# sony/timbre-trap

Hardware: AMD Instinct MI355X
Metric: audio-seconds/s training throughput (9oct x 60bpo, 3s@22.05kHz) (higher is better)
Workload: dtype bf16; 1 GPU; full train step (CQT x2 + AE fwd/bwd with consistency + 3 losses + clip + AdamW), model_complexity=2 latent=128, 64 clips x 3 s per GPU, under torch.autocast like reference experiments/train.py:415 (bf16 MFMA conv path of BASELINE config[2]; fp32 master weights, losses and optimizer); global_batch=64, parallelism=dp1

## Files before the change

timbre-trap_amd/csrc/latent_bf16.hip:

```cpp
#include "bf16_common.h"

namespace {

#ifndef LAT_WGRAD_WAVES
#define LAT_WGRAD_WAVES 4
#endif
#ifndef LAT_EXPAND_Q
#define LAT_EXPAND_Q 2
#endif
#ifndef LAT_NSPLIT
#define LAT_NSPLIT 32
#endif

__device__ __forceinline__ float gate_f(float dy, float y) { return dy * elu_dout(y); }

template <int CT> __device__ __forceinline__ int ochc(int ct, int m) { return (CT / 4) * (m >> 2) + 4 * ct + (m & 3); }

template <int CT, int DT>
__global__ __launch_bounds__(NT) void k_lat_wprep1(const float* __restrict__ w, e16* __restrict__ wp, int D, int E) {
    constexpr int SPH = CT / 32;
    const int i = blockIdx.x * NT + threadIdx.x;
    if (i >= E * SPH * DT * 64) return;
    const int lane = i & 63, dt = (i >> 6) % DT, s = (i >> 6) / DT;
    const int h = s / SPH, half = s - h * SPH;
    const int d = 16 * dt + (lane & 15), c0 = 32 * half + 8 * (lane >> 4);
    e16x8 v;
#pragma unroll
    for (int e = 0; e < 8; ++e) v[e] = (e16)(d < D ? w[((long)d * CT + c0 + e) * E + h] : 0.f);
    reinterpret_cast<e16x8*>(wp)[i] = v;
}
template <int CT, int KS>
__global__ __launch_bounds__(NT) void k_lat_wprep2(const float* __restrict__ w, e16* __restrict__ wp, int D, int E) {
    constexpr int NC = CT / 16;
    const int i = blockIdx.x * NT + threadIdx.x;
    if (i >= E * NC * KS * 64) return;
    const int lane = i & 63, s = (i >> 6) % KS, ct = ((i >> 6) / KS) % NC, h = (i >> 6) / (KS * NC);
    const int c = ochc<CT>(ct, lane & 15), d0 = 32 * s + 8 * (lane >> 4);
    e16x8 v;
#pragma unroll
    for (int e = 0; e < 8; ++e) v[e] = (e16)(d0 + e < D ? w[((long)(d0 + e) * CT + c) * E + h] : 0.f);
    reinterpret_cast<e16x8*>(wp)[i] = v;
}
template <int KS>
__global__ __launch_bounds__(NT) void k_lat_zprep(const float* __restrict__ z, e16* __restrict__ zt, int D, int Dz, float fill, int T,
                                                   long npix, float zscale, int one_row = -1) {
    constexpr int ZS = 32 * KS + 16, PCS = ZS / 8;
    const long i = (long)blockIdx.x * NT + threadIdx.x;
    const long pix = (i / (64 * PCS)) * 64 + (i & 63);
    if (pix >= npix) return;
    const int d0 = (int)((i >> 6) % PCS) * 8;
    const long b = pix / T, t = pix - b * T;
    e16x8 v;
#pragma unroll
    for (int e = 0; e < 8; ++e)
        v[e] = (e16)(zscale * (d0 + e < Dz ? z[(b * Dz + d0 + e) * T + t] : (d0 + e < D ? fill : (d0 + e == one_row ? 1.f : 0.f))));
    *reinterpret_cast<e16x8*>(zt + pix * ZS + d0) = v;
}

template <int CT, int DT, bool GATE, int QN>
__global__ __launch_bounds__(NT) void k_lat_contract(const e16* __restrict__ in, const e16* __restrict__ gy,
                                                      const e16* __restrict__ wp, const float* __restrict__ bias,
                                                      float* __restrict__ out, int D, int Dout, int E, int T, long npix, float oscale) {
    constexpr int SPH = CT / 32;
    constexpr int CHUNK = DT * 64 * 16, ROUNDS = (DT * 64 + NT - 1) / NT;
    extern __shared__ __align__(16) unsigned char smem[];
    const int tid = threadIdx.x, lane = tid & 63, wave = tid >> 6;
    const int n = lane & 15, g = lane >> 4;
    const int nsteps = E * SPH;
    const long p0 = (long)blockIdx.x * (64 * QN) + wave * (16 * QN);
    long pix[QN]; bool ok[QN]; long base[QN];
#pragma unroll
    for (int q = 0; q < QN; ++q) {
        pix[q] = p0 + 16 * q + n;
        ok[q] = pix[q] < npix;
        const long b = pix[q] / T, t = pix[q] - b * T;
        base[q] = (b * E * T + t) * CT + 8 * g;
    }
    auto stage = [&](int s, int buf) {
        const e16* src = wp + (long)s * (DT * 64 * 8);
#pragma unroll
        for (int r = 0; r < ROUNDS; ++r) {
            const int i = r * NT + wave * 64, p = i + lane;
            glds16(src + (long)(p < DT * 64 ? p : DT * 64 - 1) * 8, smem + buf * (ROUNDS * NT * 16) + (long)i * 16);
        }
    };
    auto fetch = [&](int s, e16x8 (&q8)[QN]) {
        const int h = s / SPH, half = s - h * SPH;
#pragma unroll
        for (int q = 0; q < QN; ++q) {
            const long off = base[q] + (long)h * T * CT + 32 * half;
            const bool live = ok[q] && s < nsteps;
            e16x8 v = *reinterpret_cast<const e16x8*>(in + (live ? off : 0));
            if (GATE) {
                const e16x8 yv = *reinterpret_cast<const e16x8*>(gy + (live ? off : 0));
#pragma unroll
                for (int e = 0; e < 8; ++e) v[e] = (e16)gate_f((float)v[e], (float)yv[e]);
            }
            if (!live)
#pragma unroll
                for (int e = 0; e < 8; ++e) v[e] = (e16)0.f;
            q8[q] = v;
        }
    };
    f32x4 acc[DT][QN];
#pragma unroll
    for (int dt = 0; dt < DT; ++dt)
#pragma unroll
        for (int q = 0; q < QN; ++q) acc[dt][q] = f32x4{0.f, 0.f, 0.f, 0.f};
    e16x8 bq[QN], bn[QN];
    stage(0, 0);
    fetch(0, bq);
    for (int s = 0; s < nsteps; ++s) {
        asm volatile("s_waitcnt vmcnt(0)" ::: "memory");
        __syncthreads();
        if (s + 1 < nsteps) stage(s + 1, (s + 1) & 1);
        fetch(s + 1, bn);
        const unsigned char* wb = smem + (s & 1) * (ROUNDS * NT * 16);
#pragma unroll
        for (int dt = 0; dt < DT; ++dt) {
            const e16x8 a = *reinterpret_cast<const e16x8*>(wb + ((long)dt * 64 + lane) * 16);
#pragma unroll
            for (int q = 0; q < QN; ++q) acc[dt][q] = mma32(a, bq[q], acc[dt][q]);
        }
#pragma unroll
        for (int q = 0; q < QN; ++q) bq[q] = bn[q];
    }
#pragma unroll
    for (int q = 0; q < QN; ++q) {
        if (!ok[q]) continue;
        const long b = pix[q] / T, t = pix[q] - b * T;
#pragma unroll
        for (int dt = 0; dt < DT; ++dt)
#pragma unroll
            for (int r = 0; r < 4; ++r) {
                const int d = 16 * dt + 4 * g + r;
                if (d < Dout) out[(b * Dout + d) * T + t] = acc[dt][q][r] * oscale + (bias ? bias[d] : 0.f);
            }
    }
    (void)CHUNK;
}

template <int CT, int KS, bool ACT, int QE, bool GOUT = false>
__global__ __launch_bounds__(NT) void k_lat_expand(const e16* __restrict__ zt, const e16* __restrict__ wp,
                                                    const float* __restrict__ bias, e16* __restrict__ out, int E, int T,
                                                    long npix, const e16* __restrict__ gy = nullptr) {
    constexpr int NC = CT / 16, NCH = CT / 4, ZS = 32 * KS + 16;
    constexpr int PCS = NC * KS * 64, ROUNDS = (PCS + NT - 1) / NT;
    extern __shared__ __align__(16) unsigned char smem[];
    const int tid = threadIdx.x, lane = tid & 63, wave = tid >> 6;
    const int n = lane & 15, g = lane >> 4;
    const long p0 = (long)blockIdx.x * (64 * QE) + wave * (16 * QE);
    e16x8 bz[QE][KS];
    long obase[QE]; bool ok[QE];
#pragma unroll
    for (int q = 0; q < QE; ++q) {
        const long pix = p0 + 16 * q + n;
        ok[q] = pix < npix;
        const long pc = ok[q] ? pix : 0;
#pragma unroll
        for (int s = 0; s < KS; ++s) bz[q][s] = *reinterpret_cast<const e16x8*>(zt + pc * ZS + 32 * s + 8 * g);
        const long b = pc / T, t = pc - b * T;
        obase[q] = (b * E * T + t) * CT + NCH * g;
    }
    float br[NCH];
#pragma unroll
    for (int e = 0; e < NCH; ++e) br[e] = ACT ? bias[NCH * g + e] : 0.f;
    auto stage = [&](int h, int buf) {
        const e16* src = wp + (long)h * (PCS * 8);
#pragma unroll
        for (int r = 0; r < ROUNDS; ++r) {
            const int i = r * NT + wave * 64, p = i + lane;
            glds16(src + (long)(p < PCS ? p : PCS - 1) * 8, smem + buf * (ROUNDS * NT * 16) + (long)i * 16);
        }
    };
    stage(0, 0);
    for (int h = 0; h < E; ++h) {
        asm volatile("s_waitcnt vmcnt(0)" ::: "memory");
        __syncthreads();
        if (h + 1 < E) stage(h + 1, (h + 1) & 1);
        const unsigned char* wb = smem + (h & 1) * (ROUNDS * NT * 16);
        f32x4 acc[NC][QE];
#pragma unroll
        for (int ct = 0; ct < NC; ++ct)
#pragma unroll
            for (int q = 0; q < QE; ++q) acc[ct][q] = f32x4{0.f, 0.f, 0.f, 0.f};
#pragma unroll
        for (int ct = 0; ct < NC; ++ct)
#pragma unroll
            for (int s = 0; s < KS; ++s) {
                const e16x8 a = *reinterpret_cast<const e16x8*>(wb + (((long)ct * KS + s) * 64 + lane) * 16);
#pragma unroll
                for (int q = 0; q < QE; ++q) acc[ct][q] = mma32(a, bz[q][s], acc[ct][q]);
            }
#pragma unroll
        for (int q = 0; q < QE; ++q) {
            if (!ok[q]) continue;
            e16* d = out + obase[q] + (long)h * T * CT;
#pragma unroll
            for (int c8 = 0; c8 < NCH / 8; ++c8) {
                e16x8 o, yv;
                if constexpr (GOUT) yv = *reinterpret_cast<const e16x8*>(gy + obase[q] + (long)h * T * CT + 8 * c8);
#pragma unroll
                for (int e = 0; e < 8; ++e) {
                    const int ch = 8 * c8 + e;
                    const float a = acc[ch >> 2][q][ch & 3] + br[ch];
                    o[e] = (e16)(ACT ? elu_f(a) : (GOUT ? a * elu_dout((float)yv[e]) : a));
                }
                *reinterpret_cast<e16x8*>(d + 8 * c8) = o;
            }
        }
    }
}

template <int CT> __device__ __forceinline__ int gswz(int p) { return CT == 64 ? ((p >> 1) & 3) : ((p >> 2) & 1); }

template <int CT, int DT, int KS, bool GATE>
__global__ __launch_bounds__(NT, LAT_WGRAD_WAVES) void k_lat_wgrad(const e16* __restrict__ zt, const e16* __restrict__ g_in,
                                                   const e16* __restrict__ gy, float* __restrict__ part,
                                                   float* __restrict__ dbpart, int E, int T, long npix, int nsplit) {
    constexpr int NC = CT / 16, ZS = 32 * KS + 16, ZB = ZS * 2, GB = CT * 2;
    constexpr int ZPC = 64 * ZB / 16, GPC = 64 * GB / 16;
    constexpr int ZR = (ZPC + NT - 1) / NT, GR = (GPC + NT - 1) / NT;
    constexpr int WPS = 4 / NC;
    extern __shared__ __align__(16) unsigned char smem[];
    unsigned char* zs = smem;
    unsigned char* gs = smem + ZR * NT * 16;
    const int tid = threadIdx.x, lane = tid & 63, wave = tid >> 6;
    const int n = lane & 15, g = lane >> 4, trj = n >> 2, trq = n & 3;
    const int h = blockIdx.x % E, ps = blockIdx.x / E;
    const int ct = wave % NC, sub0 = wave / NC;
    f32x4 acc[DT];
#pragma unroll
    for (int dt = 0; dt < DT; ++dt) acc[dt] = f32x4{0.f, 0.f, 0.f, 0.f};
    float dbacc[8] = {0.f, 0.f, 0.f, 0.f, 0.f, 0.f, 0.f, 0.f};
    const e16* zero = reinterpret_cast<const e16*>(&g_wzero16);
    const int npx = (int)npix, nchunks = (npx + 63) / 64;
    for (int ck = ps; ck < nchunks; ck += nsplit) {
        const int px0 = ck * 64;
        const int b0 = px0 / T, t00 = px0 - b0 * T;
        __syncthreads();
        const bool full = px0 + 64 <= npx;
        const e16* zc = zt + (long)px0 * ZS;
#pragma unroll
        for (int r = 0; r < ZR; ++r) {
            const int i = r * NT + wave * 64, p = i + lane;
            const bool okp = p < ZPC && (full || px0 + p * 16 / ZB < npx);
            glds16(okp ? zc + p * 8 : zero, zs + (long)i * 16);
        }
        e16x8 v[GATE ? GR : 1], yv[GATE ? GR : 1];
#pragma unroll
        for (int r = 0; r < GR; ++r) {
            const int i = r * NT + wave * 64, p = i + lane;
            const int q = p / (GB / 16), cgp = p % (GB / 16);
            const int cg = (((cgp >> 1) ^ gswz<CT>(q)) << 1) | (cgp & 1);
            const bool okp = p < GPC && (full || px0 + q < npx);
            int b = b0, t = t00 + q;
            if (T >= 64) { if (t >= T) { t -= T; ++b; } }
            else { const int e = t / T; b += e; t -= e * T; }
            const long off = okp ? (long)((b * E + h) * T + t) * CT + cg * 8 : 0;
            if constexpr (!GATE) glds16(okp ? g_in + off : zero, gs + (long)i * 16);
            else { v[r] = *reinterpret_cast<const e16x8*>(g_in + off); yv[r] = *reinterpret_cast<const e16x8*>(gy + off); }
        }
        if constexpr (GATE) {
#pragma unroll
            for (int r = 0; r < GR; ++r) {
                const int p = r * NT + tid;
                const bool okp = p < GPC && px0 + p / (GB / 16) < npx;
                e16x8 o;
#pragma unroll
                for (int e = 0; e < 8; ++e) {
                    const float gq = okp ? gate_f((float)v[r][e], (float)yv[r][e]) : 0.f;
                    dbacc[e] += gq;
                    o[e] = (e16)gq;
                }
                if (p < GPC) *reinterpret_cast<e16x8*>(gs + (long)p * 16) = o;
            }
        }
        asm volatile("s_waitcnt vmcnt(0)" ::: "memory");
        __syncthreads();
        for (int sub = sub0; sub < 2; sub += WPS) {
            s16x4 lo, hi;
            {
                const int p = 32 * sub + 4 * g + trj;
                lo = lds_tr16(gs + (long)p * GB + ((ct ^ gswz<CT>(p)) << 5) + 8 * trq);
                hi = lds_tr16(gs + (long)(p + 16) * GB + ((ct ^ gswz<CT>(p + 16)) << 5) + 8 * trq);
            }
            const e16x8 bq = __builtin_bit_cast(e16x8, __builtin_shufflevector(lo, hi, 0, 1, 2, 3, 4, 5, 6, 7));
#pragma unroll
            for (int dt = 0; dt < DT; ++dt) {
                const int p = 32 * sub + 4 * g + trj;
                const s16x4 alo = lds_tr16(zs + (long)p * ZB + dt * 32 + 8 * trq);
                const s16x4 ahi = lds_tr16(zs + (long)(p + 16) * ZB + dt * 32 + 8 * trq);
                acc[dt] = mma32(__builtin_bit_cast(e16x8, __builtin_shufflevector(alo, ahi, 0, 1, 2, 3, 4, 5, 6, 7)), bq, acc[dt]);
            }
        }
    }
    float* pw = part + ((long)blockIdx.x * 4 + wave) * (DT * 256);
#pragma unroll
    for (int dt = 0; dt < DT; ++dt)
#pragma unroll
        for (int r = 0; r < 4; ++r) pw[(dt * 4 + r) * 64 + lane] = acc[dt][r];
    if constexpr (GATE) {
        __syncthreads();
        float* dl = reinterpret_cast<float*>(smem);
#pragma unroll
        for (int e = 0; e < 8; ++e) dl[tid * 8 + e] = dbacc[e];
        __syncthreads();
        if (tid < CT) {
            float sum = 0.f;
            for (int t2 = 0; t2 < NT; ++t2) {
                const int q = t2 / (GB / 16), cgp = t2 % (GB / 16);
                const int cg = (((cgp >> 1) ^ gswz<CT>(q)) << 1) | (cgp & 1);
                if (cg == (tid >> 3)) sum += dl[t2 * 8 + (tid & 7)];
            }
            dbpart[(long)blockIdx.x * 64 + tid] = sum;
        }
    }
}

template <int CT, int DT>
__global__ __launch_bounds__(NT) void k_lat_wred(const float* __restrict__ part, const float* __restrict__ dbpart, float* __restrict__ dw,
                                                  float* __restrict__ db, int D, int E, int nsplit, float scale, int db_row = -1,
                                                  float* __restrict__ dbrows = nullptr) {
    constexpr int NC = CT / 16, WPS = 4 / NC, WD = DT * 256;
    const int i = blockIdx.x * NT + threadIdx.x;
    const int total = E * NC * WD;
    if (i < total) {
        const int e = i % WD, ct = (i / WD) % NC, h = i / (WD * NC);
        float sum = 0.f;
        for (int ps = 0; ps < nsplit; ++ps)
#pragma unroll
            for (int w2 = 0; w2 < WPS; ++w2) sum += part[(((long)ps * E + h) * 4 + ct + NC * w2) * WD + e];
        const int lane = e & 63, r = (e >> 6) & 3, dt = e >> 8;
        const int d = 16 * dt + 4 * (lane >> 4) + r, c = 16 * ct + (lane & 15);
        if (d < D) dw[((long)d * CT + c) * E + h] += sum * scale;
        else if (d == db_row) dbrows[h * CT + c] = sum * scale;
    } else if (db && db_row < 0 && i < total + CT * 16) {
        const int c = (i - total) % CT, sl = (i - total) / CT;
        float sum = 0.f;
        for (int wg = sl; wg < nsplit * E; wg += 16) sum += dbpart[(long)wg * 64 + c];
        atomicAdd(db + c, sum * scale);
    }
}

__global__ __launch_bounds__(64) void k_lat_dbrows(const float* __restrict__ rows, float* __restrict__ db, int E, int CT) {
    const int c = threadIdx.x;
    if (c >= CT) return;
    float t = 0.f;
    for (int h = 0; h < E; ++h) t += rows[h * CT + c];
    db[c] += t;
}

constexpr int NSPLIT = LAT_NSPLIT;

template <int CT, int DT, int KS> struct LatSizes {
    static constexpr int SPH = CT / 32, NC = CT / 16, ZS = 32 * KS + 16;
    static long wp1_bytes(int E) { return (long)E * SPH * DT * 64 * 16; }
    static long wp2_bytes(int E) { return (long)E * NC * KS * 64 * 16; }
    static long zt_bytes(long npix) { return npix * ZS * 2 + 4096; }
    static long part_bytes(int E) { return ((long)NSPLIT * E * 4 * DT * 256 + (long)NSPLIT * E * 64) * 4; }
};

template <int CT, int DT, int KS, bool GATE>
int run_contract(const e16* in, const e16* gy, const float* w, const float* bias, float* out, unsigned char* ws, int B, int D,
                 int Dout, int E, int T, hipStream_t st, bool pregated = false) {
    using L = LatSizes<CT, DT, KS>;
    const long npix = (long)B * T;
    e16* wp = reinterpret_cast<e16*>(ws);
    const int pieces = E * L::SPH * DT * 64;
    hipLaunchKernelGGL((k_lat_wprep1<CT, DT>), dim3((pieces + NT - 1) / NT), dim3(NT), 0, st, w, wp, D, E);
    TT_LAUNCH_CHECK();
    constexpr int ROUNDS = (DT * 64 + NT - 1) / NT, LDS = 2 * ROUNDS * NT * 16;
    static AttrOnce once;
#ifndef TT_LAT_QN64
#define TT_LAT_QN64 1
#endif
    constexpr int QN = CT == 64 ? TT_LAT_QN64 : 4;
    auto kern = k_lat_contract<CT, DT, GATE, QN>;
    if (int rc = raise_lds(kern, LDS, once)) return rc;
    const float oscale = (GATE || pregated) ? tt_loss_unscale() : 1.f;
    hipLaunchKernelGGL(kern, dim3((unsigned)((npix + 64 * QN - 1) / (64 * QN))), dim3(NT), LDS, st, in, gy, wp, bias, out, D, Dout, E, T, npix, oscale);
    TT_LAUNCH_CHECK();
    return 0;
}

template <int CT, int DT, int KS, bool ACT, bool GOUT = false>
int run_expand(const float* z, int Dz, float fill, const float* w, const float* bias, e16* out, unsigned char* ws, int B, int D, int E,
               int T, hipStream_t st, const e16* gy = nullptr) {
    using L = LatSizes<CT, DT, KS>;
    const long npix = (long)B * T;
    e16* wp = reinterpret_cast<e16*>(ws);
    e16* zt = reinterpret_cast<e16*>(ws + ((L::wp2_bytes(E) + 255) / 256) * 256);
    const int pieces = E * L::NC * KS * 64;
    hipLaunchKernelGGL((k_lat_wprep2<CT, KS>), dim3((pieces + NT - 1) / NT), dim3(NT), 0, st, w, wp, D, E);
    TT_LAUNCH_CHECK();
    const long zp = ((npix + 63) / 64) * 64 * (L::ZS / 8);
    hipLaunchKernelGGL((k_lat_zprep<KS>), dim3((unsigned)((zp + NT - 1) / NT)), dim3(NT), 0, st, z, zt, D, Dz, fill, T, npix,
                       ACT ? 1.f : tt_loss_scale());
    TT_LAUNCH_CHECK();
    constexpr int PCS = L::NC * KS * 64, ROUNDS = (PCS + NT - 1) / NT, LDS = 2 * ROUNDS * NT * 16;
    static AttrOnce once;
    constexpr int QE = LAT_EXPAND_Q;
    auto kern = k_lat_expand<CT, KS, ACT, QE, GOUT>;
    if (int rc = raise_lds(kern, LDS, once)) return rc;
    hipLaunchKernelGGL(kern, dim3((unsigned)((npix + 64 * QE - 1) / (64 * QE))), dim3(NT), LDS, st, zt, wp, bias, out, E, T, npix, gy);
    TT_LAUNCH_CHECK();
    return 0;
}

template <int CT, int DT, int KS, bool GATE>
int run_wgrad(const float* z, int Dz, float fill, const e16* g_in, const e16* gy, float* dw, float* db, unsigned char* ws, int B,
              int D, int E, int T, hipStream_t st, bool pregated = false) {
    using L = LatSizes<CT, DT, KS>;
    const long npix = (long)B * T;
    if (npix >= (1l << 30) || (long)B * E * T >= (1l << 31)) return TT_E_UNSUPPORTED;
    e16* zt = reinterpret_cast<e16*>(ws);
    float* part = reinterpret_cast<float*>(ws + ((L::zt_bytes(npix) + 255) / 256) * 256);
    float* dbpart = part + (long)NSPLIT * E * 4 * DT * 256;
    const long zp = ((npix + 63) / 64) * 64 * (L::ZS / 8);
    if (pregated && (GATE || D >= 16 * DT || !db)) return TT_E_UNSUPPORTED;
    const int one_row = pregated ? D : -1;
    hipLaunchKernelGGL((k_lat_zprep<KS>), dim3((unsigned)((zp + NT - 1) / NT)), dim3(NT), 0, st, z, zt, D, Dz, fill, T, npix,
                       (GATE || pregated) ? 1.f : tt_loss_scale(), one_row);
    TT_LAUNCH_CHECK();
    constexpr int ZB = L::ZS * 2, GBY = CT * 2;
    constexpr int ZR = (64 * ZB / 16 + NT - 1) / NT, GR = (64 * GBY / 16 + NT - 1) / NT;
    constexpr int LDS0 = (ZR + GR) * NT * 16, LDS = LDS0 > NT * 32 ? LDS0 : NT * 32;
    static AttrOnce once;
    auto kern = k_lat_wgrad<CT, DT, KS, GATE>;
    if (int rc = raise_lds(kern, LDS, once)) return rc;
    hipLaunchKernelGGL(kern, dim3(E * NSPLIT), dim3(NT), LDS, st, zt, g_in, gy, part, dbpart, E, T, npix, NSPLIT);
    TT_LAUNCH_CHECK();
    const int total = E * (CT / 16) * DT * 256 + CT * 16;
    hipLaunchKernelGGL((k_lat_wred<CT, DT>), dim3((total + NT - 1) / NT), dim3(NT), 0, st, part, dbpart, dw, (GATE || pregated) ? db : nullptr, D, E,
                       NSPLIT, tt_loss_unscale(), one_row, dbpart);
    TT_LAUNCH_CHECK();
    if (pregated) {
        static_assert(CT <= 64, "one wave sums the channels");
        hipLaunchKernelGGL(k_lat_dbrows, dim3(1), dim3(64), 0, st, dbpart, db, E, CT);
        TT_LAUNCH_CHECK();
    }
    return 0;
}

inline int cfg_of(int CT, int D) {
    if (CT == 32 && D >= 1 && D <= 48) return 1;
    if (CT == 64 && D >= 1 && D <= 144) return 2;
    return 0;
}

}

extern "C" {

int64_t tt_latent16_scratch_bytes(int B, int CT, int D, int E, int T) {
    const long npix = (long)B * T;
    switch (cfg_of(CT, D)) {
        case 1: { using L = LatSizes<32, 3, 2>; return L::wp1_bytes(E) + L::wp2_bytes(E) + L::zt_bytes(npix) + L::part_bytes(E) + 4096; }
        case 2: { using L = LatSizes<64, 9, 5>; return L::wp1_bytes(E) + L::wp2_bytes(E) + L::zt_bytes(npix) + L::part_bytes(E) + 4096; }
    }
    return -1;
}

int tt_latent16_contract(const void* in, const void* gy, const float* w, const float* bias, float* out, void* ws, int B, int CT, int D,
                         int Dout, int E, int T, void* stream) {
    if (!in || !w || !out || !ws || B <= 0 || E <= 0 || T <= 0 || T % 16 || Dout < 1 || Dout > D) return TT_E_BADARG;
    hipStream_t st = tt_stream(stream);
    const e16 *i = (const e16*)in, *y = (const e16*)gy;
    unsigned char* s = (unsigned char*)ws;
    switch (cfg_of(CT, D)) {
        case 1: return y ? run_contract<32, 3, 2, true>(i, y, w, bias, out, s, B, D, Dout, E, T, st) : run_contract<32, 3, 2, false>(i, y, w, bias, out, s, B, D, Dout, E, T, st);
        case 2: return y ? run_contract<64, 9, 5, true>(i, y, w, bias, out, s, B, D, Dout, E, T, st) : run_contract<64, 9, 5, false>(i, y, w, bias, out, s, B, D, Dout, E, T, st);
    }
    return TT_E_UNSUPPORTED;
}

int tt_latent16_expand(const float* z, int Dz, float fill, const float* w, const float* bias, void* out, void* ws, int B, int CT, int D,
                       int E, int T, void* stream) {
    if (!z || !w || !out || !ws || B <= 0 || E <= 0 || T <= 0 || T % 16 || (Dz != D && Dz != D - 1)) return TT_E_BADARG;
    hipStream_t st = tt_stream(stream);
    e16* o = (e16*)out;
    unsigned char* s = (unsigned char*)ws;
    switch (cfg_of(CT, D)) {
        case 1: return bias ? run_expand<32, 3, 2, true>(z, Dz, fill, w, bias, o, s, B, D, E, T, st) : run_expand<32, 3, 2, false>(z, Dz, fill, w, bias, o, s, B, D, E, T, st);
        case 2: return bias ? run_expand<64, 9, 5, true>(z, Dz, fill, w, bias, o, s, B, D, E, T, st) : run_expand<64, 9, 5, false>(z, Dz, fill, w, bias, o, s, B, D, E, T, st);
    }
    return TT_E_UNSUPPORTED;
}

int tt_latent16_wgrad(const float* z, int Dz, float fill, const void* g, const void* gy, float* dw, float* db, void* ws, int B, int CT,
                      int D, int E, int T, void* stream) {
    if (!z || !g || !dw || !ws || (gy && !db) || B <= 0 || E <= 0 || T <= 0 || T % 16 || (Dz != D && Dz != D - 1)) return TT_E_BADARG;
    hipStream_t st = tt_stream(stream);
    const e16 *gi = (const e16*)g, *y = (const e16*)gy;
    unsigned char* s = (unsigned char*)ws;
    switch (cfg_of(CT, D)) {
        case 1: return y ? run_wgrad<32, 3, 2, true>(z, Dz, fill, gi, y, dw, db, s, B, D, E, T, st) : run_wgrad<32, 3, 2, false>(z, Dz, fill, gi, y, dw, db, s, B, D, E, T, st);
        case 2: return y ? run_wgrad<64, 9, 5, true>(z, Dz, fill, gi, y, dw, db, s, B, D, E, T, st) : run_wgrad<64, 9, 5, false>(z, Dz, fill, gi, y, dw, db, s, B, D, E, T, st);
    }
    return TT_E_UNSUPPORTED;
}

int tt_latent16_pregated_ok(int CT, int D) {
    switch (cfg_of(CT, D)) {
        case 1: return D < 16 * 3;
        case 2: return D < 16 * 9;
    }
    return 0;
}

int tt_latent16_expand_gated(const float* z, const float* w, const void* gy, void* out, void* ws, int B, int CT, int D, int E, int T,
                             void* stream) {
    if (!z || !w || !gy || !out || !ws || B <= 0 || E <= 0 || T <= 0 || T % 16) return TT_E_BADARG;
    hipStream_t st = tt_stream(stream);
    switch (cfg_of(CT, D)) {
        case 1: return run_expand<32, 3, 2, false, true>(z, D, 0.f, w, nullptr, (e16*)out, (unsigned char*)ws, B, D, E, T, st, (const e16*)gy);
        case 2: return run_expand<64, 9, 5, false, true>(z, D, 0.f, w, nullptr, (e16*)out, (unsigned char*)ws, B, D, E, T, st, (const e16*)gy);
    }
    return TT_E_UNSUPPORTED;
}

int tt_latent16_contract_pregated(const void* g, const float* w, float* out, void* ws, int B, int CT, int D, int Dout, int E, int T,
                                  void* stream) {
    if (!g || !w || !out || !ws || B <= 0 || E <= 0 || T <= 0 || T % 16 || Dout < 1 || Dout > D) return TT_E_BADARG;
    hipStream_t st = tt_stream(stream);
    switch (cfg_of(CT, D)) {
        case 1: return run_contract<32, 3, 2, false>((const e16*)g, nullptr, w, nullptr, out, (unsigned char*)ws, B, D, Dout, E, T, st, true);
        case 2: return run_contract<64, 9, 5, false>((const e16*)g, nullptr, w, nullptr, out, (unsigned char*)ws, B, D, Dout, E, T, st, true);
    }
    return TT_E_UNSUPPORTED;
}

int tt_latent16_wgrad_pregated(const float* z, int Dz, float fill, const void* g, float* dw, float* db, void* ws, int B, int CT, int D,
                               int E, int T, void* stream) {
    if (!z || !g || !dw || !db || !ws || B <= 0 || E <= 0 || T <= 0 || T % 16 || (Dz != D && Dz != D - 1)) return TT_E_BADARG;
    hipStream_t st = tt_stream(stream);
    switch (cfg_of(CT, D)) {
        case 1: return run_wgrad<32, 3, 2, false>(z, Dz, fill, (const e16*)g, nullptr, dw, db, (unsigned char*)ws, B, D, E, T, st, true);
        case 2: return run_wgrad<64, 9, 5, false>(z, Dz, fill, (const e16*)g, nullptr, dw, db, (unsigned char*)ws, B, D, E, T, st, true);
    }
    return TT_E_UNSUPPORTED;
}

}
```

Before: 3838 audio-seconds/s.

## Add pipelined latent contract, expand, and paired-head wgrad kernels

Adds a multi-stage prefetch contract kernel that streams activation tiles into LDS several steps ahead with counted vmcnt waits instead of full drains. The expand kernel gets a pipelined variant that waits only for the weight stage while output stores stay in flight, and hoists the gradient loads and ELU derivative. A new non-gated wgrad kernel processes two heads per block so the z tile is loaded once for both. All three are enabled by default through a schedule switch, at the cost of more LDS per block and lower occupancy.

```diff
diff --git a/timbre-trap_amd/csrc/latent_bf16.hip b/timbre-trap_amd/csrc/latent_bf16.hip
--- a/timbre-trap_amd/csrc/latent_bf16.hip
+++ b/timbre-trap_amd/csrc/latent_bf16.hip
@@ -140,7 +140,112 @@
     (void)CHUNK;
 }
 
-template <int CT, int KS, bool ACT, int QE, bool GOUT = false>
+#ifndef LAT_CONTRACT_PF
+#define LAT_CONTRACT_PF 4
+#endif
+constexpr int lat_contract_pf(bool gate) { return gate && LAT_CONTRACT_PF > 4 ? 4 : LAT_CONTRACT_PF; }
+template <int CT, int DT, bool GATE, int QN>
+__global__ __launch_bounds__(NT) void k_lat_contract_pipe(const e16* __restrict__ in, const e16* __restrict__ gy,
+                                                           const e16* __restrict__ wp, const float* __restrict__ bias,
+                                                           float* __restrict__ out, int D, int Dout, int E, int T, long npix, float oscale) {
+    constexpr int SPH = CT / 32, PF = lat_contract_pf(GATE);
+    constexpr int ROUNDS = (DT * 64 + NT - 1) / NT, BUFB = ROUNDS * NT * 16, SLOTB = 4 * QN * 1024;
+    constexpr int NLD = QN * (GATE ? 2 : 1);
+    static_assert(PF >= 3 && NLD < 64, "the operand of step s must be older than stage(s); vmcnt has six bits");
+    extern __shared__ __align__(16) unsigned char smem[];
+    unsigned char* xs = smem + 2 * BUFB;
+    unsigned char* ys = xs + PF * SLOTB;
+    const int tid = threadIdx.x, lane = tid & 63, wave = tid >> 6;
+    const int n = lane & 15, g = lane >> 4;
+    const int nsteps = E * SPH;
+    const long p0 = (long)blockIdx.x * (64 * QN) + wave * (16 * QN);
+    long pix[QN]; bool ok[QN]; long base[QN];
+#pragma unroll
+    for (int q = 0; q < QN; ++q) {
+        pix[q] = p0 + 16 * q + n;
+        ok[q] = pix[q] < npix;
+        const long pc = ok[q] ? pix[q] : 0;
+        const long b = pc / T, t = pc - b * T;
+        base[q] = (b * E * T + t) * CT + 8 * g;
+    }
+    auto stage = [&](int s, int buf) {
+        const e16* src = wp + (long)s * (DT * 64 * 8);
+#pragma unroll
+        for (int r = 0; r < ROUNDS; ++r) {
+            const int i = r * NT + wave * 64, p = i + lane;
+            glds16(src + (long)(p < DT * 64 ? p : DT * 64 - 1) * 8, smem + buf * BUFB + (long)i * 16);
+        }
+    };
+    auto request = [&](int s, int slot) {
+        const int sc = s < nsteps ? s : nsteps - 1;
+        const int h = sc / SPH, half = sc - h * SPH;
+#pragma unroll
+        for (int q = 0; q < QN; ++q) {
+            const long off = base[q] + (long)h * T * CT + 32 * half;
+            const int o = slot * SLOTB + (wave * QN + q) * 1024;
+            glds16(in + off, xs + o);
+            if (GATE) glds16(gy + off, ys + o);
+        }
+    };
+    f32x4 acc[DT][QN];
+#pragma unroll
+    for (int dt = 0; dt < DT; ++dt)
+#pragma unroll
+        for (int q = 0; q < QN; ++q) acc[dt][q] = f32x4{0.f, 0.f, 0.f, 0.f};
+#pragma unroll
+    for (int j = 0; j < PF - 2; ++j) request(j, j);
+    stage(0, 0);
+    request(PF - 2, PF - 2);
+    int slot = 0;
+    for (int s = 0; s < nsteps; ++s) {
+        asm volatile("s_waitcnt vmcnt(%0) lgkmcnt(0)\n\ts_barrier" ::"n"(NLD) : "memory");
+        if (s + 1 < nsteps) stage(s + 1, (s + 1) & 1);
+        request(s + PF - 1, slot == 0 ? PF - 1 : slot - 1);
+        asm volatile("" ::: "memory");
+        e16x8 bq[QN];
+#pragma unroll
+        for (int q = 0; q < QN; ++q) {
+            const int o = slot * SLOTB + (wave * QN + q) * 1024 + lane * 16;
+            bq[q] = *reinterpret_cast<const e16x8*>(xs + o);
+            if (GATE) {
+                const e16x8 yv = *reinterpret_cast<const e16x8*>(ys + o);
+#pragma unroll
+                for (int e = 0; e < 8; ++e) bq[q][e] = (e16)gate_f((float)bq[q][e], (float)yv[e]);
+            }
+        }
+        const unsigned char* wb = smem + (s & 1) * BUFB;
+#pragma unroll
+        for (int dt = 0; dt < DT; ++dt) {
+            const e16x8 a = *reinterpret_cast<const e16x8*>(wb + ((long)dt * 64 + lane) * 16);
+#pragma unroll
+            for (int q = 0; q < QN; ++q) acc[dt][q] = mma32(a, bq[q], acc[dt][q]);
+        }
+        slot = slot + 1 == PF ? 0 : slot + 1;
+    }
+    asm volatile("s_waitcnt vmcnt(0)" ::: "memory");
+    float bv[DT][4];
+#pragma unroll
+    for (int dt = 0; dt < DT; ++dt)
+#pragma unroll
+        for (int r = 0; r < 4; ++r) {
+            const int d = 16 * dt + 4 * g + r;
+            bv[dt][r] = (bias && d < Dout) ? bias[d] : 0.f;
+        }
+#pragma unroll
+    for (int q = 0; q < QN; ++q) {
+        if (!ok[q]) continue;
+        const long b = pix[q] / T, t = pix[q] - b * T;
+#pragma unroll
+        for (int dt = 0; dt < DT; ++dt)
+#pragma unroll
+            for (int r = 0; r < 4; ++r) {
+                const int d = 16 * dt + 4 * g + r;
+                if (d < Dout) out[(b * Dout + d) * T + t] = acc[dt][q][r] * oscale + bv[dt][r];
+            }
+    }
+}
+
+template <int CT, int KS, bool ACT, int QE, bool GOUT = false, bool PIPE = false>
 __global__ __launch_bounds__(NT) void k_lat_expand(const e16* __restrict__ zt, const e16* __restrict__ wp,
                                                     const float* __restrict__ bias, e16* __restrict__ out, int E, int T,
                                                     long npix, const e16* __restrict__ gy = nullptr) {
@@ -173,11 +278,31 @@
             glds16(src + (long)(p < PCS ? p : PCS - 1) * 8, smem + buf * (ROUNDS * NT * 16) + (long)i * 16);
         }
     };
+    constexpr int NST = QE * (NCH / 8);
+    bool allok = true;
+#pragma unroll
+    for (int q = 0; q < QE; ++q) allok = allok && ok[q];
+    const bool counted = PIPE && __builtin_amdgcn_readfirstlane((int)allok) != 0;
     stage(0, 0);
     for (int h = 0; h < E; ++h) {
-        asm volatile("s_waitcnt vmcnt(0)" ::: "memory");
-        __syncthreads();
+        if constexpr (PIPE) {
+            if (counted && h > 0) asm volatile("s_waitcnt vmcnt(%0) lgkmcnt(0)\n\ts_barrier" ::"n"(NST) : "memory");
+            else asm volatile("s_waitcnt vmcnt(0) lgkmcnt(0)\n\ts_barrier" ::: "memory");
+        } else {
+            asm volatile("s_waitcnt vmcnt(0)" ::: "memory");
+            __syncthreads();
+        }
+        e16x8 yv[QE][NCH / 8];
+        if constexpr (GOUT && PIPE) {
+#pragma unroll
+            for (int q = 0; q < QE; ++q)
+#pragma unroll
+                for (int c8 = 0; c8 < NCH / 8; ++c8)
+                    yv[q][c8] = *reinterpret_cast<const e16x8*>(gy + obase[q] + (long)h * T * CT + 8 * c8);
+            asm volatile("" ::: "memory");
+        }
         if (h + 1 < E) stage(h + 1, (h + 1) & 1);
+        if constexpr (PIPE) asm volatile("" ::: "memory");
         const unsigned char* wb = smem + (h & 1) * (ROUNDS * NT * 16);
         f32x4 acc[NC][QE];
 #pragma unroll
@@ -192,19 +317,30 @@
 #pragma unroll
                 for (int q = 0; q < QE; ++q) acc[ct][q] = mma32(a, bz[q][s], acc[ct][q]);
             }
+        float gf[GOUT && PIPE ? QE : 1][GOUT && PIPE ? NCH : 1];
+        if constexpr (GOUT && PIPE) {
+            __builtin_amdgcn_sched_barrier(0);
+#pragma unroll
+            for (int q = 0; q < QE; ++q)
+#pragma unroll
+                for (int ch = 0; ch < NCH; ++ch) {
+                    gf[q][ch] = elu_dout((float)yv[q][ch >> 3][ch & 7]);
+                    asm volatile("" : "+v"(gf[q][ch]));
+                }
+        }
 #pragma unroll
         for (int q = 0; q < QE; ++q) {
             if (!ok[q]) continue;
             e16* d = out + obase[q] + (long)h * T * CT;
 #pragma unroll
             for (int c8 = 0; c8 < NCH / 8; ++c8) {
-                e16x8 o, yv;
-                if constexpr (GOUT) yv = *reinterpret_cast<const e16x8*>(gy + obase[q] + (long)h * T * CT + 8 * c8);
+                e16x8 o;
+                if constexpr (GOUT && !PIPE) yv[q][c8] = *reinterpret_cast<const e16x8*>(gy + obase[q] + (long)h * T * CT + 8 * c8);
 #pragma unroll
                 for (int e = 0; e < 8; ++e) {
                     const int ch = 8 * c8 + e;
                     const float a = acc[ch >> 2][q][ch & 3] + br[ch];
-                    o[e] = (e16)(ACT ? elu_f(a) : (GOUT ? a * elu_dout((float)yv[e]) : a));
+                    o[e] = (e16)(ACT ? elu_f(a) : (GOUT ? a * (PIPE ? gf[GOUT && PIPE ? q : 0][GOUT && PIPE ? ch : 0] : elu_dout((float)yv[q][c8][e])) : a));
                 }
                 *reinterpret_cast<e16x8*>(d + 8 * c8) = o;
             }
@@ -318,6 +454,88 @@
     }
 }
 
+template <int CT, int DT, int KS>
+__global__ __launch_bounds__(NT, 2) void k_lat_wgrad_hp(const e16* __restrict__ zt, const e16* __restrict__ g_in, float* __restrict__ part,
+                                                         int E, int T, long npix, int nsplit) {
+    constexpr int NC = CT / 16, ZS = 32 * KS + 16, ZB = ZS * 2, GB = CT * 2;
+    constexpr int ZPC = 64 * ZB / 16, GPC = 64 * GB / 16;
+    constexpr int ZR = (ZPC + NT - 1) / NT, GR = (GPC + NT - 1) / NT;
+    constexpr int WPS = 4 / NC;
+    extern __shared__ __align__(16) unsigned char smem[];
+    unsigned char* zs = smem;
+    unsigned char* gs = smem + ZR * NT * 16;
+    const int tid = threadIdx.x, lane = tid & 63, wave = tid >> 6;
+    const int n = lane & 15, g = lane >> 4, trj = n >> 2, trq = n & 3;
+    const int nhp = (E + 1) / 2;
+    const int hp = blockIdx.x % nhp, ps = blockIdx.x / nhp;
+    const int h0 = 2 * hp;
+    const bool two = h0 + 1 < E;
+    const int ct = wave % NC, sub0 = wave / NC;
+    f32x4 acc[2][DT];
+#pragma unroll
+    for (int hh = 0; hh < 2; ++hh)
+#pragma unroll
+        for (int dt = 0; dt < DT; ++dt) acc[hh][dt] = f32x4{0.f, 0.f, 0.f, 0.f};
+    const e16* zero = reinterpret_cast<const e16*>(&g_wzero16);
+    const int npx = (int)npix, nchunks = (npx + 63) / 64;
+    for (int ck = ps; ck < nchunks; ck += nsplit) {
+        const int px0 = ck * 64;
+        const int b0 = px0 / T, t00 = px0 - b0 * T;
+        __syncthreads();
+        const bool full = px0 + 64 <= npx;
+        const e16* zc = zt + (long)px0 * ZS;
+#pragma unroll
+        for (int r = 0; r < ZR; ++r) {
+            const int i = r * NT + wave * 64, p = i + lane;
+            const bool okp = p < ZPC && (full || px0 + p * 16 / ZB < npx);
+            glds16(okp ? zc + p * 8 : zero, zs + (long)i * 16);
+        }
+#pragma unroll
+        for (int r = 0; r < GR; ++r) {
+            const int i = r * NT + wave * 64, p = i + lane;
+            const int q = p / (GB / 16), cgp = p % (GB / 16);
+            const int cg = (((cgp >> 1) ^ gswz<CT>(q)) << 1) | (cgp & 1);
+            const bool okp = p < GPC && (full || px0 + q < npx);
+            int b = b0, t = t00 + q;
+            if (T >= 64) { if (t >= T) { t -= T; ++b; } }
+            else { const int e = t / T; b += e; t -= e * T; }
+            const long off = okp ? (long)((b * E + h0) * T + t) * CT + cg * 8 : 0;
+            glds16(okp ? g_in + off : zero, gs + (long)i * 16);
+            if (two) glds16(okp ? g_in + off + (long)T * CT : zero, gs + GR * NT * 16 + (long)i * 16);
+        }
+        asm volatile("s_waitcnt vmcnt(0)" ::: "memory");
+        __syncthreads();
+        for (int sub = sub0; sub < 2; sub += WPS) {
+            const int p = 32 * sub + 4 * g + trj;
+            e16x8 bq[2];
+#pragma unroll
+            for (int hh = 0; hh < 2; ++hh) {
+                const unsigned char* gh = gs + hh * (GR * NT * 16);
+                const s16x4 lo = lds_tr16(gh + (long)p * GB + ((ct ^ gswz<CT>(p)) << 5) + 8 * trq);
+                const s16x4 hi = lds_tr16(gh + (long)(p + 16) * GB + ((ct ^ gswz<CT>(p + 16)) << 5) + 8 * trq);
+                bq[hh] = __builtin_bit_cast(e16x8, __builtin_shufflevector(lo, hi, 0, 1, 2, 3, 4, 5, 6, 7));
+            }
+#pragma unroll
+            for (int dt = 0; dt < DT; ++dt) {
+                const s16x4 alo = lds_tr16(zs + (long)p * ZB + dt * 32 + 8 * trq);
+                const s16x4 ahi = lds_tr16(zs + (long)(p + 16) * ZB + dt * 32 + 8 * trq);
+                const e16x8 a = __builtin_bit_cast(e16x8, __builtin_shufflevector(alo, ahi, 0, 1, 2, 3, 4, 5, 6, 7));
+                acc[0][dt] = mma32(a, bq[0], acc[0][dt]);
+                if (two) acc[1][dt] = mma32(a, bq[1], acc[1][dt]);
+            }
+        }
+    }
+#pragma unroll
+    for (int hh = 0; hh < 2; ++hh) {
+        if (hh == 1 && !two) break;
+        float* pw = part + (((long)ps * E + h0 + hh) * 4 + wave) * (DT * 256);
+#pragma unroll
+        for (int dt = 0; dt < DT; ++dt)
+#pragma unroll
+            for (int r = 0; r < 4; ++r) pw[(dt * 4 + r) * 64 + lane] = acc[hh][dt][r];
+    }
+}
+
 template <int CT, int DT>
 __global__ __launch_bounds__(NT) void k_lat_wred(const float* __restrict__ part, const float* __restrict__ dbpart, float* __restrict__ dw,
                                                   float* __restrict__ db, int D, int E, int nsplit, float scale, int db_row = -1,
@@ -353,6 +571,11 @@
 
 constexpr int NSPLIT = LAT_NSPLIT;
 
+#ifndef TT_LAT_SCHED
+#define TT_LAT_SCHED 7
+#endif
+inline int lat_sched() { return tt_switch("TTRAP_LAT_SCHED", TT_LAT_SCHED); }
+
 template <int CT, int DT, int KS> struct LatSizes {
     static constexpr int SPH = CT / 32, NC = CT / 16, ZS = 32 * KS + 16;
     static long wp1_bytes(int E) { return (long)E * SPH * DT * 64 * 16; }
@@ -371,14 +594,25 @@
     hipLaunchKernelGGL((k_lat_wprep1<CT, DT>), dim3((pieces + NT - 1) / NT), dim3(NT), 0, st, w, wp, D, E);
     TT_LAUNCH_CHECK();
     constexpr int ROUNDS = (DT * 64 + NT - 1) / NT, LDS = 2 * ROUNDS * NT * 16;
-    static AttrOnce once;
+    static AttrOnce once, once_p;
 #ifndef TT_LAT_QN64
 #define TT_LAT_QN64 1
 #endif
+#ifndef TT_LAT_QN64P
+#define TT_LAT_QN64P 4
+#endif
+    const float oscale = (GATE || pregated) ? tt_loss_unscale() : 1.f;
+    if (lat_sched() & 1) {
+        constexpr int QP = CT == 64 ? TT_LAT_QN64P : 2, LDSP = 2 * ROUNDS * NT * 16 + (GATE ? 2 : 1) * lat_contract_pf(GATE) * 4 * QP * 1024;
+        auto kern = k_lat_contract_pipe<CT, DT, GATE, QP>;
+        if (int rc = raise_lds(kern, LDSP, once_p)) return rc;
+        hipLaunchKernelGGL(kern, dim3((unsigned)((npix + 64 * QP - 1) / (64 * QP))), dim3(NT), LDSP, st, in, gy, wp, bias, out, D, Dout, E, T, npix, oscale);
+        TT_LAUNCH_CHECK();
+        return 0;
+    }
     constexpr int QN = CT == 64 ? TT_LAT_QN64 : 4;
     auto kern = k_lat_contract<CT, DT, GATE, QN>;
     if (int rc = raise_lds(kern, LDS, once)) return rc;
-    const float oscale = (GATE || pregated) ? tt_loss_unscale() : 1.f;
     hipLaunchKernelGGL(kern, dim3((unsigned)((npix + 64 * QN - 1) / (64 * QN))), dim3(NT), LDS, st, in, gy, wp, bias, out, D, Dout, E, T, npix, oscale);
     TT_LAUNCH_CHECK();
     return 0;
@@ -399,8 +633,15 @@
                        ACT ? 1.f : tt_loss_scale());
     TT_LAUNCH_CHECK();
     constexpr int PCS = L::NC * KS * 64, ROUNDS = (PCS + NT - 1) / NT, LDS = 2 * ROUNDS * NT * 16;
-    static AttrOnce once;
+    static AttrOnce once, once_p;
     constexpr int QE = LAT_EXPAND_Q;
+    if (lat_sched() & 2) {
+        auto kern = k_lat_expand<CT, KS, ACT, QE, GOUT, true>;
+        if (int rc = raise_lds(kern, LDS, once_p)) return rc;
+        hipLaunchKernelGGL(kern, dim3((unsigned)((npix + 64 * QE - 1) / (64 * QE))), dim3(NT), LDS, st, zt, wp, bias, out, E, T, npix, gy);
+        TT_LAUNCH_CHECK();
+        return 0;
+    }
     auto kern = k_lat_expand<CT, KS, ACT, QE, GOUT>;
     if (int rc = raise_lds(kern, LDS, once)) return rc;
     hipLaunchKernelGGL(kern, dim3((unsigned)((npix + 64 * QE - 1) / (64 * QE))), dim3(NT), LDS, st, zt, wp, bias, out, E, T, npix, gy);
@@ -426,11 +667,19 @@
     constexpr int ZB = L::ZS * 2, GBY = CT * 2;
     constexpr int ZR = (64 * ZB / 16 + NT - 1) / NT, GR = (64 * GBY / 16 + NT - 1) / NT;
     constexpr int LDS0 = (ZR + GR) * NT * 16, LDS = LDS0 > NT * 32 ? LDS0 : NT * 32;
-    static AttrOnce once;
-    auto kern = k_lat_wgrad<CT, DT, KS, GATE>;
-    if (int rc = raise_lds(kern, LDS, once)) return rc;
-    hipLaunchKernelGGL(kern, dim3(E * NSPLIT), dim3(NT), LDS, st, zt, g_in, gy, part, dbpart, E, T, npix, NSPLIT);
-    TT_LAUNCH_CHECK();
+    static AttrOnce once, once_p;
+    if (!GATE && (lat_sched() & 4)) {
+        constexpr int LDSP = (ZR + 2 * GR) * NT * 16;
+        auto kern = k_lat_wgrad_hp<CT, DT, KS>;
+        if (int rc = raise_lds(kern, LDSP, once_p)) return rc;
+        hipLaunchKernelGGL(kern, dim3(((E + 1) / 2) * NSPLIT), dim3(NT), LDSP, st, zt, g_in, part, E, T, npix, NSPLIT);
+        TT_LAUNCH_CHECK();
+    } else {
+        auto kern = k_lat_wgrad<CT, DT, KS, GATE>;
+        if (int rc = raise_lds(kern, LDS, once)) return rc;
+        hipLaunchKernelGGL(kern, dim3(E * NSPLIT), dim3(NT), LDS, st, zt, g_in, gy, part, dbpart, E, T, npix, NSPLIT);
+        TT_LAUNCH_CHECK();
+    }
     const int total = E * (CT / 16) * DT * 256 + CT * 16;
     hipLaunchKernelGGL((k_lat_wred<CT, DT>), dim3((total + NT - 1) / NT), dim3(NT), 0, st, part, dbpart, dw, (GATE || pregated) ? db : nullptr, D, E,
                        NSPLIT, tt_loss_unscale(), one_row, dbpart);
```

Result: no change. 3843 audio-seconds/s (median of 6 runs) (+0.1%).
